# d8ahazard/AudioLab

Hardware: AMD Instinct MI355X
Metric: stems*realtime-factor (44.1kHz stereo) (higher is better)
Workload: dtype bf16; 1 GPU; MDX-Net UVR 4-stem (4x TFC-TDF U-Net L=11 g=48 dim_f=3072 dim_t=256 n_fft=6144), 300 s 44.1 kHz stereo in total, margin chunker, windows/launch=52; stems=4

## Files before the change

### audiolab_amd/csrc/tdfnet.hip

```cpp
#include "mma.h"
#include <alsep_gfx950_asm.h>

#include <map>
#include <type_traits>

namespace {

constexpr int kThreads = 256;

template <typename T> struct Vec16;
template <> struct Vec16<float> { static constexpr int N = 4; };
template <> struct Vec16<bf16_t> { static constexpr int N = 8; };
__device__ __forceinline__ void store_vec(float* p, const float* y) { *reinterpret_cast<float4*>(p) = make_float4(y[0], y[1], y[2], y[3]); }
__device__ __forceinline__ void store_vec(bf16_t* p, const float* y) {
    bf16x8 q;
#pragma unroll
    for (int e = 0; e < 8; ++e) q[e] = (bf16_t)y[e];
    *reinterpret_cast<bf16x8*>(p) = q;
}
__device__ __forceinline__ void load_vec(const float* p, float* x) {
    const float4 q = *reinterpret_cast<const float4*>(p);
    x[0] = q.x; x[1] = q.y; x[2] = q.z; x[3] = q.w;
}
__device__ __forceinline__ void load_vec(const bf16_t* p, float* x) {
// ... 2357 lines not shown
#pragma unroll
    for (int j = 0; j < P::D; ++j)
        if (j < nmy) issue(j);
    for (int i = 0; i < nmy; ++i) {
        pipe_wait_tile<P::D, P::ND, P::NS>(i, nmy);
        barrier_nodrain();
        if (i + P::D < nmy) issue(i + P::D);
        if (i > 0) copy_out(i - 1);
        const bf16_t* xs = reinterpret_cast<const bf16_t*>(xring + (size_t)(i % P::NSX) * P::x_bytes);
        f32x4 acc[P::MT][P::NI];
#pragma unroll
        for (int mt = 0; mt < P::MT; ++mt)
#pragma unroll
            for (int ni = 0; ni < P::NI; ++ni) acc[mt][ni] = f32x4{0.f, 0.f, 0.f, 0.f};
        bf16x8 xf[2][P::NI];
        static_for<P::NI>([&](auto nic) {
            constexpr int ni = decltype(nic)::value;
            lds_read_async_b128<ni * 2 * P::XREG>(xf[0][ni], xs + bk[0] / sizeof(bf16_t));
        });
        static_for<P::KS>([&](auto ksc) {
            constexpr int ks = decltype(ksc)::value, b = ks & 1;
            if constexpr (ks + 1 < P::KS) {
                static_for<P::NI>([&](auto nic) {
                    constexpr int ni = decltype(nic)::value;
                    lds_read_async_b128<ni * 2 * P::XREG>(xf[1 - b][ni], xs + bk[ks + 1] / sizeof(bf16_t));
                });
                lds_wait_n<P::NI>();
            } else {
                lds_wait_n<0>();
                if (P::C % 32 != 0) {
#pragma unroll
                    for (int ni = 0; ni < P::NI; ++ni) xf[b][ni] = klast_ok ? xf[b][ni] : bf16x8{};
                }
            }
#pragma unroll
            for (int mt = 0; mt < P::MT; ++mt)
#pragma unroll
                for (int ni = 0; ni < P::NI; ++ni) mma_step(acc[mt][ni], wf[mt][ks], xf[b][ni]);
        });
        bf16_t* sl = reinterpret_cast<bf16_t*>(sring + (size_t)(i % P::NSS) * P::s_bytes + ebase);
        const float* bnl = bn + 4 * lq;
        auto eoff = [&](int mt) {
            int t = 2 * mt + erot;
            t = t >= P::NG ? t - P::NG : t;
            return t * 8;
        };
        bf16x8 ev[2][P::NI];
        f32x4 scv[2], shv[2];
        auto eread = [&](auto mtc) {
            constexpr int mt = decltype(mtc)::value, eb = mt & 1;
            const bf16_t* p = sl + eoff(mt);
            static_for<P::NI>([&](auto nic) {
                constexpr int ni = decltype(nic)::value;
                lds_read_async_b128<ni * 32 * P::NG * 16>(ev[eb][ni], p);
            });
            lds_read_async_f32x4<0>(scv[eb], bnl + mt * 16);
            lds_read_async_f32x4<P::C2 * 4>(shv[eb], bnl + mt * 16);
        };
        eread(std::integral_constant<int, 0>{});
        static_for<P::MT>([&](auto mtc) {
            constexpr int mt = decltype(mtc)::value, b = mt & 1;
            if constexpr (mt + 1 < P::MT) {
                eread(std::integral_constant<int, mt + 1>{});
                lds_wait_n<P::NI + 2>();
            } else {
                lds_wait_n<0>();
            }
            bf16_t* p = sl + eoff(mt) + (lq & 1) * 4;
            static_for<P::NI>([&](auto nic) {
                constexpr int ni = decltype(nic)::value;
                const bf16x4 sk = (lq & 1) ? __builtin_shufflevector(ev[b][ni], ev[b][ni], 4, 5, 6, 7)
                                           : __builtin_shufflevector(ev[b][ni], ev[b][ni], 0, 1, 2, 3);
                bf16x4 q;
#pragma unroll
                for (int r = 0; r < 4; ++r) q[r] = (bf16_t)(fmaxf(fmaf(acc[mt][ni][r], scv[b][r], shv[b][r]), 0.f) * (float)sk[r]);
                lds_write_async_b64(p + ni * 32 * P::NG * 8, q);
            });
        });
    }
    barrier_nodrain();
    copy_out(nmy - 1);
}

template <int NM_, int TW_>
struct ConvAllco {
    static constexpr int NM = NM_, TW = TW_, TH = 8, KC = 48, CG = 6, NG = 54, NS = 14, NI = TW / 16, ROWS = 16 * NM, NB = NM, NPAIR = NB / 2;
    static constexpr int UPK = NM % 4 == 0 ? 4 : 3, G = NM / UPK;
    static constexpr int KS = 1, NSLOT = 4, DIST = NSLOT - 1, NSTG = NS / KS, UPS = UPK * KS;
    static constexpr int PW = TW + 2, PH = TH + 2;
    static constexpr int PGROUPS = PH * PW * CG, PINST = (PGROUPS + 63) / 64, PJ = (PINST + 7) / 8, PBUF = PINST * 64;
    static constexpr int KSTEP_BYTES = ROWS * 64, SLOT_BYTES = KS * KSTEP_BYTES;
    static constexpr int WPW = SLOT_BYTES / 8;
    static constexpr int WJ = (WPW + 1023) / 1024, WLAST = (WPW - (WJ - 1) * 1024) / 16;
    static constexpr int ST = NI * (NPAIR + NB % 2);
    static constexpr size_t ring_bytes = 16 * (size_t)(2 * PBUF) + (size_t)NSLOT * SLOT_BYTES;
    static constexpr size_t lds_bytes = ring_bytes + 2 * ROWS * sizeof(float) + 1024;
    static_assert(NM % 3 == 0 && NM % UPK == 0 && TW % 16 == 0 && NS % KS == 0 && SLOT_BYTES % (8 * 16) == 0, "ConvAllco: shape");
    static_assert(DIST >= 2 && DIST < NSTG && WJ < UPS && PJ - 1 <= NSTG - DIST && NSTG - 1 >= PJ, "ConvAllco: DMA schedule");
    static_assert(lds_bytes <= 160 * 1024, "ConvAllco: LDS budget");
    __host__ __device__ static constexpr int wswz(int row) { return ((row >> 3) & 1) << 1; }
    __host__ __device__ static constexpr int tapoff(int tap) { return ((tap / 3) * PW + tap % 3) * KC * 2; }
    __host__ __device__ static constexpr int xconst(int st) { return tapoff(4 * st / CG) + 16 * (4 * st % CG); }
    __host__ __device__ static constexpr int xkind(int st) { return st == 4 ? 1 : st == NS - 1 ? 2 : 0; }
    __host__ __device__ static constexpr int xbase(int kind, int wave, int l15, int lq) {
        const int a = (wave * PW + l15) * KC * 2 + 16 * lq;
        return kind == 0 ? a : kind == 1 ? a + (lq >= 2 ? (PW - 3) * KC * 2 : 0) : a - (lq >= 2 ? 16 * (lq - 1) : 0);
    }
    static_assert(CG == 6 && NS == 14 && NG == 54, "xconst / xkind are written for 54 groups in 14 k-steps");
    __host__ __device__ static constexpr int dma_of_stage(int sc) { return WJ + (sc < PJ ? 1 : 0); }
    __host__ __device__ static constexpr int inflight_at(int sc) {
        int n = 0;
        for (int i = 1; i <= DIST - 2; ++i) n += dma_of_stage((sc - i + NSTG) % NSTG);
        return n;
    }
};

template <typename Cf, int U>
__device__ __forceinline__ void allco_read_w(bf16x8 (&wf)[2][Cf::G], const bf16_t* wl) {
    constexpr int st = U / Cf::UPK, t = U % Cf::UPK;
    static_for<Cf::G>([&](auto gc) {
        constexpr int g = decltype(gc)::value;
        lds_read_async_b128<(t * Cf::G + g) * 1024 + (st % Cf::KS) * Cf::KSTEP_BYTES>(wf[U & 1][g], wl);
    });
}
template <typename Cf, int ST, int NI>
__device__ __forceinline__ void allco_read_x(bf16x8& xf, const bf16_t* pb) {
    lds_read_async_b128<NI * 16 * Cf::KC * 2 + Cf::xconst(ST)>(xf, pb);
}

template <int NM, int TW>
__global__ void __launch_bounds__(kBigThreads, 2)
conv3x3_bf16_allco_kernel(const bf16_t* __restrict__ X, bf16_t* __restrict__ Y, const bf16_t* __restrict__ Wp, const float* __restrict__ scale,
                          const float* __restrict__ shift, const bf16_t* __restrict__ zero_page, int Th, int Fw, int Cin, int Cout, int tiles_t,
                          int tiles_f, int ntiles) {
    typedef ConvAllco<NM, TW> Cf;
    bf16_t* const patch0 = reinterpret_cast<bf16_t*>(alsep_smem);
    bf16_t* const wring = patch0 + (size_t)2 * Cf::PBUF * 8;
    float* ss = reinterpret_cast<float*>(alsep_smem + Cf::ring_bytes);
    bf16_t* const scratch = reinterpret_cast<bf16_t*>(alsep_smem + Cf::lds_bytes - 1024);
    const int tid = threadIdx.x, lane = tid & 63, wave = __builtin_amdgcn_readfirstlane(tid >> 6);
    const int l15 = lane & 15, lq = lane >> 4;
    const int nq = Cin / Cf::KC;
    for (int i = tid; i < Cf::ROWS; i += kBigThreads) {
        ss[i] = scale[i];
        ss[Cf::ROWS + i] = shift[i];
    }
    __syncthreads();

    int xb[3];
#pragma unroll
    for (int kind = 0; kind < 3; ++kind) xb[kind] = Cf::xbase(kind, wave, l15, lq) / 2;
    const int wl_off = l15 * 32 + (lq ^ Cf::wswz(l15)) * 8;

    const int my_tiles = (ntiles - (int)blockIdx.x + (int)gridDim.x - 1) / (int)gridDim.x;
    const int npatch = my_tiles * nq;
    auto tile_coords = [&](int k, int& t0, int& f0, int64_t& b) {
        int tile = (int)blockIdx.x + k * (int)gridDim.x;
        const int tf = tile % tiles_f;  tile /= tiles_f;
        const int tt = tile % tiles_t;
        b = tile / tiles_t;
        t0 = tt * Cf::TH;
        f0 = tf * Cf::TW;
    };
    int prel[Cf::PJ];
    unsigned pflags[(Cf::PJ + 5) / 6] = {};
#pragma unroll
    for (int j = 0; j < Cf::PJ; ++j) {
        const int u = (wave + 8 * j) * 64 + lane;
        const int uu = u < Cf::PGROUPS ? u : Cf::PGROUPS - 1;
        const int P = uu / Cf::CG, cg = uu % Cf::CG;
        const int dt = P / Cf::PW - 1, df = P % Cf::PW - 1;
        prel[j] = (dt * Fw + df) * Cin + cg * 8;
        pflags[j / 6] |= (u < Cf::PGROUPS ? (unsigned)((dt < 0) | ((dt >= Cf::TH) << 1) | ((df < 0) << 2) | ((df >= Cf::TW) << 3)) : 16u) << (5 * (j % 6));
    }
    const bf16_t* psrc = X;
    unsigned pborder = 0;
    bf16_t* pdst = patch0;
    auto patch_prep = [&](int ps) {
        const int pc = ps < npatch ? ps : npatch - 1;
        int t0, f0; int64_t b;
        tile_coords(pc / nq, t0, f0, b);
        psrc = X + ((b * Th + t0) * (int64_t)Fw + f0) * Cin + (pc % nq) * Cf::KC;
        pborder = (unsigned)(t0 == 0) | ((unsigned)(t0 + Cf::TH >= Th) << 1) | ((unsigned)(f0 == 0) << 2) | ((unsigned)(f0 + Cf::TW >= Fw) << 3);
        pdst = patch0 + (size_t)(ps & 1) * Cf::PBUF * 8;
    };
    auto patch_one = [&](int j) {
        const int i = wave + 8 * j;
        const bool out = (pflags[j / 6] & ((pborder | 16u) << (5 * (j % 6)))) != 0;
        const bool real = j < Cf::PJ - 1 || i < Cf::PINST;
        const bf16_t* src = (out || !real) ? zero_page : psrc + opaque_vgpr(prel[j]);
        glds16(src, real ? pdst + (size_t)i * 64 * 8 : scratch);
    };
    const unsigned wlane = lane * 8;
    const bf16_t* wsrc_next = Wp;
    bf16_t* wdst_next = wring;
    auto weights_prep = [&](int q, int sc, int slot) {
        wsrc_next = Wp + ((size_t)q * Cf::NSTG + sc) * (Cf::SLOT_BYTES / 2) + wave * (Cf::WPW / 2);
        wdst_next = wring + (size_t)slot * (Cf::SLOT_BYTES / 2) + wave * (Cf::WPW / 2);
    };
    auto weights_one = [&](int j) {
        if (j < Cf::WJ - 1 || Cf::WLAST == 64 || lane < Cf::WLAST) glds16(wsrc_next + (wlane + j * 512u), wdst_next + j * 512);
    };

    f32x4 acc[Cf::NB][Cf::NI];
    bf16x8 xf[Cf::NI], wf[2][Cf::G];
    auto read_first = [&](const bf16_t* patch, const bf16_t* wl) {
        allco_read_w<Cf, 0>(wf, wl);
        static_for<Cf::NI>([&](auto nic) { allco_read_x<Cf, 0, decltype(nic)::value>(xf[decltype(nic)::value], patch + xb[0]); });
    };
    if (npatch > 0) {
        patch_prep(0);
#pragma unroll
        for (int j = 0; j < Cf::PJ; ++j) patch_one(j);
#pragma unroll
        for (int d = 0; d < Cf::DIST; ++d) {
            weights_prep(0, d, d);
#pragma unroll
            for (int j = 0; j < Cf::WJ; ++j) weights_one(j);
        }
        wait_vmcnt<0>();
        barrier_nodrain();
        read_first(patch0, wring + wl_off);
    }
    auto epilogue = [&](int k) {
        int t0, f0; int64_t b;
        tile_coords(k, t0, f0, b);
        const int le = opaque_vgpr(lane), l15 = le & 15, lq = le >> 4;
        bf16_t* yb = Y + ((b * Th + t0 + wave) * (int64_t)Fw + f0 + l15) * Cout;
#pragma unroll
        for (int j = 0; j < Cf::NPAIR; ++j) {
            const int co = j * 32 + lq * 8;
            f32x4 scv[2], shv[2];
#pragma unroll
            for (int h = 0; h < 2; ++h) {
                scv[h] = *reinterpret_cast<const f32x4*>(ss + co + 4 * h);
                shv[h] = *reinterpret_cast<const f32x4*>(ss + Cf::ROWS + co + 4 * h);
            }
#pragma unroll
            for (int ni = 0; ni < Cf::NI; ++ni) {
                float y[8];
#pragma unroll
                for (int h = 0; h < 2; ++h)
#pragma unroll
                    for (int r = 0; r < 4; ++r) y[4 * h + r] = fmaxf(fmaf(acc[2 * j + h][ni][r], scv[h][r], shv[h][r]), 0.f);
                store8(yb + (int64_t)ni * 16 * Cout + co, y);
            }
        }
        if constexpr (Cf::NB % 2 == 1) {
            constexpr int bb = Cf::NB - 1;
            const int co = bb * 16 + lq * 4;
            const f32x4 scv = *reinterpret_cast<const f32x4*>(ss + co);
            const f32x4 shv = *reinterpret_cast<const f32x4*>(ss + Cf::ROWS + co);
#pragma unroll
            for (int ni = 0; ni < Cf::NI; ++ni) {
                float y[4];
#pragma unroll
                for (int r = 0; r < 4; ++r) y[r] = fmaxf(fmaf(acc[bb][ni][r], scv[r], shv[r]), 0.f);
                store4(yb + (int64_t)ni * 16 * Cout + co, y);
            }
        }
    };

    int slot = 0, q = 0, k = 0;
    for (int p = 0; p < npatch; ++p) {
        const bf16_t* const patch = patch0 + (size_t)(p & 1) * Cf::PBUF * 8;
        const bf16_t* const patch_nx = patch0 + (size_t)((p + 1) & 1) * Cf::PBUF * 8;
        const int qn = q + 1 == nq ? 0 : q + 1;
        static_for<Cf::NSTG>([&](auto scc) {
            constexpr int sc = decltype(scc)::value;
            if (sc < Cf::DIST - 1 && q == 0 && p > 0) wait_vmcnt<Cf::inflight_at(sc) + Cf::ST>();
            else wait_vmcnt<Cf::inflight_at(sc)>();
            __builtin_amdgcn_s_barrier();
            const int slot_prev = slot == 0 ? Cf::NSLOT - 1 : slot - 1, slot_nx = slot + 1 == Cf::NSLOT ? 0 : slot + 1;
            weights_prep((sc + Cf::DIST) / Cf::NSTG ? qn : q, (sc + Cf::DIST) % Cf::NSTG, slot_prev);
            if (sc == 0) {
                patch_prep(p + 1);
                if (q == 0) {
#pragma unroll
                    for (int b = 0; b < Cf::NB; ++b)
#pragma unroll
                        for (int ni = 0; ni < Cf::NI; ++ni) acc[b][ni] = f32x4{0.f, 0.f, 0.f, 0.f};
                }
            }
            const bf16_t* const wl = wring + (size_t)slot * (Cf::SLOT_BYTES / 2) + wl_off;
            const bf16_t* const wl_nx = wring + (size_t)slot_nx * (Cf::SLOT_BYTES / 2) + wl_off;
            static_for<Cf::UPS>([&](auto uic) {
                constexpr int ui = decltype(uic)::value, U = sc * Cf::UPS + ui, t = U % Cf::UPK, st = U / Cf::UPK;
                constexpr bool chunk_end = U + 1 == Cf::UPK * Cf::NS;
                constexpr int U1 = chunk_end ? 0 : U + 1, st1 = U1 / Cf::UPK;
                if constexpr (t == 0) lds_wait_n<Cf::NI - 1>();
                else lds_wait_n<0>();
                if constexpr (!chunk_end) allco_read_w<Cf, U1>(wf, ui + 1 < Cf::UPS ? wl : wl_nx);
                if constexpr (t == 0) {
                    static_for<Cf::NI>([&](auto nic) {
                        constexpr int ni = decltype(nic)::value;
                        if constexpr (ni > 0) lds_wait_n<Cf::G + Cf::NI - 1 - ni>();
#pragma unroll
                        for (int g = 0; g < Cf::G; ++g) mma_step(acc[t * Cf::G + g][ni], wf[U & 1][g], xf[ni]);
                    });
                } else if constexpr (t == Cf::UPK - 1 && !chunk_end) {
                    const bf16_t* const pb = patch + xb[Cf::xkind(st1)];
                    static_for<Cf::NI>([&](auto nic) {
                        constexpr int ni = decltype(nic)::value;
#pragma unroll
                        for (int g = 0; g < Cf::G; ++g) mma_step(acc[t * Cf::G + g][ni], wf[U & 1][g], xf[ni]);
                        sched_fence();
                        allco_read_x<Cf, st1, ni>(xf[ni], pb);
                    });
                } else {
#pragma unroll
                    for (int g = 0; g < Cf::G; ++g)
#pragma unroll
                        for (int ni = 0; ni < Cf::NI; ++ni) mma_step(acc[t * Cf::G + g][ni], wf[U & 1][g], xf[ni]);
                }
                if constexpr (ui < Cf::WJ) weights_one(ui);
                if constexpr (ui == Cf::WJ && sc < Cf::PJ) patch_one(sc);
                sched_fence();
            });
            slot = slot_nx;
            if (sc == Cf::NSTG - 1 && q == nq - 1) epilogue(k);
        });
        read_first(patch_nx, wring + (size_t)slot * (Cf::SLOT_BYTES / 2) + wl_off);
        q = qn;
        if (q == 0) ++k;
    }
    lds_wait_n<0>();
    wait_vmcnt<0>();
}

#ifndef ALSEP_F16_TU
#include "tdfnet_f32s.h"
#endif

struct DevBuf {
    void* p = nullptr;
    size_t bytes = 0;
};

struct ConvLayer {
    DevBuf w, scale, shift;
    DevBuf w_big;
    DevBuf w_mq;
    DevBuf w_ac;
    int cin = 0, cout = 0;
    bool dma_path = false;
    int split = 0;
    unsigned* range_flag = nullptr;
};
struct GemmLayer {
    DevBuf w, bias, scale, shift;
    int M = 0, K = 0, Kp = 0, Mp = 0;
    bool has_bias = false;
    bool split = false;
    unsigned* range_flag = nullptr;
    bool dma_path = false;
    DevBuf wfrag;
    DevBuf wwide;
};
struct Block {
    std::vector<ConvLayer> tfc;
    std::vector<GemmLayer> tdf;
};

}

struct alsep_net {
    alsep_ctx* ctx = nullptr;
    alsep_net_config cfg{};
    int n = 0;
    bool split = false;
    DevBuf range_flag;
    std::vector<DevBuf> owned;
    DevBuf first_w, first_scale, first_shift, final_w, final_b, zero_page;
    std::vector<Block> enc, dec;
    Block bott;
    std::vector<GemmLayer> ds, us;
};

namespace {

typedef std::map<std::string, std::vector<float>> TensorMap;

template <typename T> T host_cast(float v);
template <> float host_cast<float>(float v) { return v; }
template <> bf16_t host_cast<bf16_t>(float v) { return (bf16_t)v; }

int upload(alsep_net* net, const void* src, size_t bytes, DevBuf* out) {
    void* d = nullptr;
    if (hipMalloc(&d, bytes ? bytes : 16) != hipSuccess) return alsep_fail(net->ctx, ALSEP_ERR_NOMEM, "hipMalloc(%zu) failed", bytes);
    out->p = d;
    out->bytes = bytes;
    net->owned.push_back(*out);
    if (bytes) ALSEP_HIP(net->ctx, hipMemcpy(d, src, bytes, hipMemcpyHostToDevice));
    return ALSEP_OK;
}

const std::vector<float>* find(const TensorMap& tm, const std::string& name, int64_t numel, alsep_ctx* ctx, bool required = true) {
    auto it = tm.find(name);
    if (it == tm.end()) {
        if (required) alsep_fail(ctx, ALSEP_ERR_ARG, "missing tensor '%s'", name.c_str());
        return nullptr;
    }
    if ((int64_t)it->second.size() != numel) {
        alsep_fail(ctx, ALSEP_ERR_ARG, "tensor '%s' has %zu elements, expected %lld", name.c_str(), it->second.size(), (long long)numel);
        return nullptr;
    }
    return &it->second;
// ... 54 lines not shown
    for (int R = 0; R < cout; ++R) std::copy(w.begin() + ConvBig<NY>::channel_of_row(R) * row, w.begin() + (ConvBig<NY>::channel_of_row(R) + 1) * row, wp.begin() + R * row);
    return pack_conv3x3_dma(wp, cin, cout);
}

std::vector<bf16_t> pack_conv3x3_mq(const std::vector<float>& w, int cin) {
    typedef ConvMq Cf;
    const int nq = cin / Cf::KC;
    std::vector<bf16_t> out((size_t)nq * Cf::PARTS * Cf::WGROUPS * 8, host_cast<bf16_t>(0.f));
    for (int q = 0; q < nq; ++q)
        for (int pt = 0; pt < Cf::PARTS; ++pt)
            for (int R = 0; R < Cf::ROWS; ++R)
                for (int stl = 0; stl < Cf::ksteps_of_part(pt); ++stl)
                    for (int lq = 0; lq < 4; ++lq) {
                        const int tap = pt * Cf::KS + stl, co = ConvBig<2>::channel_of_row(R);
                        const size_t dst = ((((size_t)q * Cf::PARTS + pt) * Cf::ROWS + R) * Cf::WG + 4 * stl + (lq ^ Cf::wswz(R))) * 8;
                        for (int e = 0; e < 8; ++e) {
                            const int ci = q * Cf::KC + lq * 8 + e;
                            out[dst + e] = host_cast<bf16_t>(w[(((size_t)co * cin + ci) * 3 + tap / 3) * 3 + tap % 3]);
                        }
                    }
    return out;
}

template <int NM>
std::vector<bf16_t> pack_conv3x3_allco(const std::vector<float>& w, int cin) {
    typedef ConvAllco<NM, 48> Cf;
    const int nq = cin / Cf::KC;
    std::vector<bf16_t> out((size_t)nq * Cf::NS * Cf::ROWS * 32, host_cast<bf16_t>(0.f));
    for (int q = 0; q < nq; ++q)
        for (int st = 0; st < Cf::NS; ++st)
            for (int R = 0; R < Cf::ROWS; ++R)
                for (int lq = 0; lq < 4; ++lq) {
                    const int grp = 4 * st + lq;
                    if (grp >= Cf::NG) continue;
                    const int tap = grp / Cf::CG, cg = grp % Cf::CG, co = ConvBig<NM / 3>::channel_of_row(R);
                    const size_t dst = ((((size_t)q * Cf::NS + st) * Cf::ROWS + R) * 4 + (lq ^ Cf::wswz(R))) * 8;
                    for (int e = 0; e < 8; ++e) {
                        const int ci = q * Cf::KC + cg * 8 + e;
                        out[dst + e] = host_cast<bf16_t>(w[(((size_t)co * cin + ci) * 3 + tap / 3) * 3 + tap % 3]);
                    }
                }
    return out;
}

template <typename T> constexpr bool is_bf16() { return false; }
template <> constexpr bool is_bf16<bf16_t>() { return true; }

template <typename T>
int make_conv(alsep_net* net, const TensorMap& tm, const std::string& p, int c, ConvLayer* L) {
    auto w = find(tm, p + ".weight", (int64_t)c * c * 9, net->ctx);
    auto sc = find(tm, p + ".scale", c, net->ctx);
    auto sh = find(tm, p + ".shift", c, net->ctx);
    if (!w || !sc || !sh) return ALSEP_ERR_ARG;
    L->cin = L->cout = c;
    int rc;
#ifndef ALSEP_F16_TU
    if (!is_bf16<T>() && net->split && (c % 48 == 0 || c % 16 == 0)) {
        L->split = c % 48 == 0 ? 24 : 16;
        L->range_flag = (unsigned*)net->range_flag.p;
        const std::vector<hs_t> pk = L->split == 24 ? pack_conv3x3_split<24, 48>(*w, c, c) : pack_conv3x3_split<16, 16>(*w, c, c);
        rc = upload(net, pk.data(), pk.size() * sizeof(hs_t), &L->w);
    } else
#endif
    if (is_bf16<T>() && c % 48 == 0) {
        L->dma_path = true;
        auto pk = pack_conv3x3_dma(*w, c, c);
        rc = upload(net, pk.data(), pk.size() * sizeof(bf16_t), &L->w);
        if (!rc && c == 48) {
            auto p0 = pack_conv3x3_big<1>(*w, c);
            rc = upload(net, p0.data(), p0.size() * sizeof(bf16_t), &L->w_big);
        }
        if (!rc && c == 96) {
            auto pq = pack_conv3x3_mq(*w, c);
            rc = upload(net, pq.data(), pq.size() * sizeof(bf16_t), &L->w_mq);
        }
        if (!rc && c == 144) {
            auto pb = pack_conv3x3_big<3>(*w, c);
            rc = upload(net, pb.data(), pb.size() * sizeof(bf16_t), &L->w_big);
        }
        if (!rc && c == 144) {
            auto pa = pack_conv3x3_allco<9>(*w, c);
            rc = upload(net, pa.data(), pa.size() * sizeof(bf16_t), &L->w_ac);
        }
    } else if (conv_uses_main<T>(c, c)) {
        auto pk = pack_conv3x3<T, ConvSel<T>::KC, ConvSel<T>::BN>(*w, c, c);
        rc = upload(net, pk.data(), pk.size() * sizeof(T), &L->w);
    } else {
        auto pk = pack_conv3x3<T, ConvSel16<T>::KC, ConvSel16<T>::BN>(*w, c, c);
        rc = upload(net, pk.data(), pk.size() * sizeof(T), &L->w);
    }
    if (rc) return rc;
    if ((rc = upload(net, sc->data(), c * sizeof(float), &L->scale))) return rc;
    return upload(net, sh->data(), c * sizeof(float), &L->shift);
}

template <typename T>
int make_gemm_weights(alsep_net* net, const std::vector<float>& wmk, int M, int K, GemmLayer* L) {
    typedef GemmCfg<T> Gc;
    L->M = M; L->K = K;
#ifndef ALSEP_F16_TU
    if (!is_bf16<T>() && net->split) {
        L->split = true;
        L->range_flag = (unsigned*)net->range_flag.p;
        const std::vector<hs_t> pk = pack_gemm_split(wmk, M, K, &L->Mp, &L->Kp);
        return upload(net, pk.data(), pk.size() * sizeof(hs_t), &L->w);
    }
#endif
    L->Mp = (int)ceil_div64(M, Gc::BR) * Gc::BR;
    L->Kp = (int)ceil_div64(K, Gc::BK) * Gc::BK;
    std::vector<T> pk((size_t)L->Mp * L->Kp, host_cast<T>(0.f));
    for (int m = 0; m < M; ++m)
        for (int k = 0; k < K; ++k) pk[(size_t)m * L->Kp + k] = host_cast<T>(wmk[(size_t)m * K + k]);
    return upload(net, pk.data(), pk.size() * sizeof(T), &L->w);
}

int make_tdf_dma_weights(alsep_net* net, const std::vector<float>& wmk, int M, int K, GemmLayer* L) {
    typedef TdfB16 Tc;
    L->M = M; L->K = K;
    L->Mp = (int)ceil_div64(M, Tc::BM) * Tc::BM;
    L->Kp = (int)ceil_div64(K, Tc::BK) * Tc::BK;
    L->dma_path = true;
    std::vector<bf16_t> pk((size_t)L->Mp * L->Kp, host_cast<bf16_t>(0.f));
    for (int m = 0; m < M; ++m)
        for (int kt = 0; kt < L->Kp / Tc::BK; ++kt)
            for (int g = 0; g < 8; ++g) {
                const int ks = g >> 2, lq = g & 3, pg = g ^ ((m >> 1) & 7);
                for (int e = 0; e < 8; ++e) {
                    const int k = kt * Tc::BK + ks * 32 + (e < 4 ? 4 * lq + e : 16 + 4 * lq + (e - 4));
                    if (k < K) pk[(size_t)m * L->Kp + kt * Tc::BK + pg * 8 + e] = host_cast<bf16_t>(wmk[(size_t)m * K + k]);
                }
            }
    return upload(net, pk.data(), pk.size() * sizeof(bf16_t), &L->w);
}

int make_tdf_wide_weights(alsep_net* net, const std::vector<float>& wmk, int M, int K, GemmLayer* L) {
    const int KT = (int)ceil_div64(K, 64);
    std::vector<bf16_t> pk((size_t)(M / 48) * KT * 6 * 512, host_cast<bf16_t>(0.f));
    for (int rb = 0; rb < M / 48; ++rb)
        for (int kt = 0; kt < KT; ++kt)
            for (int ks = 0; ks < 2; ++ks)
                for (int mi = 0; mi < 3; ++mi)
                    for (int l = 0; l < 64; ++l)
                        for (int e = 0; e < 8; ++e) {
                            const int lq = l >> 4, m = rb * 48 + mi * 16 + (l & 15);
                            const int k = kt * 64 + ks * 32 + (e < 4 ? 4 * lq + e : 16 + 4 * lq + (e - 4));
                            if (k < K)
                                pk[((((size_t)rb * KT + kt) * 2 + ks) * 3 + mi) * 512 + l * 8 + e] =
                                    host_cast<bf16_t>(wmk[(size_t)m * K + k]);
                        }
    return upload(net, pk.data(), pk.size() * sizeof(bf16_t), &L->wwide);
}

int make_frag_weights(alsep_net* net, const std::vector<float>& wmk, int M, int K, DevBuf* out) {
    const int MT = (M + 15) / 16, KS = (K + 31) / 32;
    std::vector<bf16_t> pk((size_t)MT * KS * 64 * 8, host_cast<bf16_t>(0.f));
    for (int mt = 0; mt < MT; ++mt)
        for (int ks = 0; ks < KS; ++ks)
            for (int l = 0; l < 64; ++l)
                for (int e = 0; e < 8; ++e) {
                    const int m = mt * 16 + (l & 15), k = ks * 32 + (l >> 4) * 8 + e;
                    if (m < M && k < K) pk[(((size_t)mt * KS + ks) * 64 + l) * 8 + e] = host_cast<bf16_t>(wmk[(size_t)m * K + k]);
                }
    return upload(net, pk.data(), pk.size() * sizeof(bf16_t), out);
}

template <typename T>
// ... 131 lines not shown
    typedef ConvB16<TW> Cf;
    const int tiles_t = (int)ceil_div64(Th, Cf::TH), tiles_f = (int)ceil_div64(Fw, TW);
    const int64_t ntiles = B * tiles_t * tiles_f;
    if (ntiles > 0x7fffffff) return alsep_fail(ctx, ALSEP_ERR_ARG, "conv3x3: too many tiles");
    ALSEP_HIP(ctx, hipFuncSetAttribute((const void*)conv3x3_bf16_kernel<TW>, hipFuncAttributeMaxDynamicSharedMemorySize,
                                       (int)Cf::lds_bytes));
    ProfScope prof(ctx, TW == 64 ? ALSEP_PROF_CONV3X3 : ALSEP_PROF_CONV3X3_SMALL);
    prof.work(18.0 * (double)L.cin * L.cout * B * Th * Fw, (double)sizeof(*X) * B * Th * Fw * (L.cin + L.cout));
    const int nyc = L.cout / Cf::BN;
    const int ny_fastest = conv_ny_fastest() && ntiles % 8 == 0 && nyc > 1 && ntiles * nyc <= 0x7fffffff;
    hipLaunchKernelGGL((conv3x3_bf16_kernel<TW>), ny_fastest ? dim3((unsigned)(ntiles * nyc)) : dim3((unsigned)ntiles, nyc),
                       dim3(kThreads), Cf::lds_bytes,
                       ctx->stream, X, Y, (const bf16_t*)L.w.p, (const float*)L.scale.p, (const float*)L.shift.p, zero_page,
                       Th, Fw, L.cin, L.cout, tiles_t, tiles_f, (int)ntiles,  0,  0, ny_fastest);
    note_launch(ctx, TW == 64 ? "conv3x3_bf16_kernel<64>" : "conv3x3_bf16_kernel<small>");
    ALSEP_LAUNCH_CHECK(ctx, "conv3x3_bf16_kernel");
    return ALSEP_OK;
}

template <int NQ, int RING_ = 3, int OCC = 1, int TW_ = 64>
int launch_conv_regw(alsep_ctx* ctx, const ConvLayer& L, const bf16_t* X, bf16_t* Y, const bf16_t* zero_page, int64_t B,
                     int Th, int Fw) {
    typedef ConvRW<NQ, RING_, TW_> Cf;
    const int tiles_t = Th / Cf::TH, tiles_f = Fw / Cf::TW;
    const int64_t ntiles = B * tiles_t * tiles_f;
    if (ntiles > 0x7fffffff) return alsep_fail(ctx, ALSEP_ERR_ARG, "conv3x3: too many tiles");
    ALSEP_HIP(ctx, hipFuncSetAttribute((const void*)conv3x3_bf16_regw_kernel<NQ, RING_, OCC, TW_>,
                                       hipFuncAttributeMaxDynamicSharedMemorySize, (int)Cf::lds_bytes));
    const int ny = L.cout / Cf::BN;
    int gx = OCC * 256 / ny;
    if (gx > ntiles) gx = (int)ntiles;
    ProfScope prof(ctx, ALSEP_PROF_CONV3X3_REGW);
    prof.work(18.0 * (double)L.cin * L.cout * B * Th * Fw, (double)sizeof(*X) * B * Th * Fw * (L.cin + L.cout));
    hipLaunchKernelGGL((conv3x3_bf16_regw_kernel<NQ, RING_, OCC, TW_>), dim3((unsigned)gx, ny), dim3(kThreads), Cf::lds_bytes, ctx->stream, X, Y,
                       (const bf16_t*)L.w.p, (const float*)L.scale.p, (const float*)L.shift.p, zero_page, Th, Fw, L.cin,
                       L.cout, tiles_t, tiles_f, (int)ntiles);
    ALSEP_LAUNCH_CHECK(ctx, "conv3x3_bf16_regw_kernel");
    return ALSEP_OK;
}

template <typename Cf, typename Kern>
int launch_conv_persist(alsep_ctx* ctx, Kern kern, const ConvLayer& L, const DevBuf& wimg, int prof_class, const char* name, const bf16_t* X,
                        bf16_t* Y, const bf16_t* zero_page, int64_t B, int Th, int Fw, int grid_cap = 0) {
    const int tiles_t = Th / Cf::TH, tiles_f = Fw / Cf::TW;
    const int64_t ntiles = B * tiles_t * tiles_f;
    if (ntiles > 0x7fffffff) return alsep_fail(ctx, ALSEP_ERR_ARG, "conv3x3: too many tiles");
    ALSEP_HIP(ctx, hipFuncSetAttribute((const void*)kern, hipFuncAttributeMaxDynamicSharedMemorySize, (int)Cf::lds_bytes));
    int gx = ntiles < 256 ? (int)ntiles : 256;
    if (grid_cap > 0 && gx > grid_cap) gx = grid_cap;
    ProfScope prof(ctx, prof_class);
    prof.work(18.0 * (double)L.cin * L.cout * B * Th * Fw, (double)sizeof(*X) * B * Th * Fw * (L.cin + L.cout));
    hipLaunchKernelGGL(kern, dim3((unsigned)gx), dim3(kBigThreads), Cf::lds_bytes, ctx->stream, X, Y, (const bf16_t*)wimg.p,
                       (const float*)L.scale.p, (const float*)L.shift.p, zero_page, Th, Fw, L.cin, L.cout, tiles_t, tiles_f, (int)ntiles);
    ALSEP_LAUNCH_CHECK(ctx, name);
    return ALSEP_OK;
}

int launch_conv_big3(alsep_ctx* ctx, const ConvLayer& L, const bf16_t* X, bf16_t* Y, const bf16_t* zero_page, int64_t B, int Th, int Fw) {
    if (!L.w_big.p) return alsep_fail(ctx, ALSEP_ERR_STATE, "conv3x3: no big-tile weight image for this layer");
    if (int rc = launch_conv_persist<ConvBig<3>>(ctx, conv3x3_bf16_big_kernel<3>, L, L.w_big, ALSEP_PROF_CONV3X3_BIG3, "conv3x3_bf16_big_kernel",
                                                 X, Y, zero_page, B, Th, Fw))
        return rc;
    note_launch(ctx, "conv3x3_bf16_big_kernel<3>");
    return ALSEP_OK;
}

int launch_conv_mq(alsep_ctx* ctx, const ConvLayer& L, const bf16_t* X, bf16_t* Y, const bf16_t* zero_page, int64_t B, int Th, int Fw) {
    if (!L.w_mq.p || L.cout != ConvMq::ROWS || L.cin % ConvMq::KC) return alsep_fail(ctx, ALSEP_ERR_STATE, "conv3x3: no mq weight image for this layer");
    return launch_conv_persist<ConvMq>(ctx, conv3x3_bf16_mq_kernel, L, L.w_mq, ALSEP_PROF_CONV3X3_BIG, "conv3x3_bf16_mq_kernel", X, Y, zero_page,
                                       B, Th, Fw);
}

int launch_conv_m0(alsep_ctx* ctx, const ConvLayer& L, const bf16_t* X, bf16_t* Y, const bf16_t* zero_page, int64_t B, int Th, int Fw) {
    if (!L.w_big.p || L.cout != ConvM0::ROWS || L.cin != ConvM0::KC) return alsep_fail(ctx, ALSEP_ERR_STATE, "conv3x3: no m0 weight image for this layer");
    return launch_conv_persist<ConvM0>(ctx, conv3x3_bf16_m0_kernel, L, L.w_big, ALSEP_PROF_CONV3X3_REGW, "conv3x3_bf16_m0_kernel", X, Y, zero_page,
                                       B, Th, Fw);
}

int conv_allco_grid() {
    static const int v = env_int("ALSEP_CONV_ALLCO_GRID", 0);
    return v;
}

template <int NM>
int launch_conv_allco(alsep_ctx* ctx, const ConvLayer& L, const bf16_t* X, bf16_t* Y, const bf16_t* zero_page, int64_t B, int Th, int Fw) {
    typedef ConvAllco<NM, 48> Cf;
    if (!L.w_ac.p || L.cout != Cf::ROWS || L.cin != L.cout) return alsep_fail(ctx, ALSEP_ERR_STATE, "conv3x3: no all-channels weight image for this layer");
    static_assert(NM == 9, "only the c = 144 instance is shipped: the profiling class and the names below are level 2's");
    if (int rc = launch_conv_persist<Cf>(ctx, conv3x3_bf16_allco_kernel<NM, 48>, L, L.w_ac, ALSEP_PROF_CONV3X3_BIG3, "conv3x3_bf16_allco_kernel", X, Y,
                                         zero_page, B, Th, Fw, conv_allco_grid()))
        return rc;
    note_launch(ctx, "conv3x3_bf16_big_kernel");
    note_launch(ctx, "conv3x3_bf16_big_kernel<3>");
    return ALSEP_OK;
}

int conv_m0_enabled() {
    static const int v = env_int("ALSEP_CONV_M0", 1);
    return v;
}
int conv_regw_enabled() {
    static const int v = env_int("ALSEP_CONV_REGW", 1);
    return v;
}
int conv_big_enabled() {
    static const int v = env_int("ALSEP_CONV_BIG", 1);
    return v;
}
int conv_mq_enabled() {
    static const int v = env_int("ALSEP_CONV_MQ", 1);
    return v;
}
int conv_big3_enabled() {
    static const int v = env_int("ALSEP_CONV_BIG3", 1);
    return v;
}

int conv_allco_enabled() {
    static const int v = env_int("ALSEP_CONV_ALLCO", 1);
    return v;
}
constexpr int kConvAllco144 = 1;
constexpr int kConvAllcoRouted = kConvAllco144;

int run_conv_dma(alsep_ctx* ctx, const ConvLayer& L, const bf16_t* X, bf16_t* Y, const bf16_t* zp, int64_t B, int Th, int Fw) {
    if (conv_m0_enabled() && L.cin == 48 && L.cout == 48 && Th % 8 == 0 && Fw % 48 == 0 &&
        (conv_m0_enabled() >= 2 || B * (Th / 8) * (Fw / 48) >= 256))
        return launch_conv_m0(ctx, L, X, Y, zp, B, Th, Fw);
    if (conv_regw_enabled() && Th % 4 == 0 && Fw % 64 == 0 && L.cin == L.cout) {
        if (L.cin == 48 && conv_regw_enabled() == 3) return launch_conv_regw<1>(ctx, L, X, Y, zp, B, Th, Fw);
        if (L.cin == 48) return launch_conv_regw<1, 3, 2, 32>(ctx, L, X, Y, zp, B, Th, Fw);
        if (L.cin == 96 && conv_regw_enabled() >= 2) return launch_conv_regw<2>(ctx, L, X, Y, zp, B, Th, Fw);
    }
    if (conv_big_enabled() && conv_big3_enabled() && conv_allco_enabled() && Th % 8 == 0 && Fw % 48 == 0 && L.cin == 144 && L.cout == 144) {
        const int mode = conv_allco_enabled();
        const bool big3_shape = Fw % 64 == 0 && (conv_big_enabled() >= 2 || B * (Th / 8) * (Fw / 64) >= 96);
        if (mode >= 2 || ((kConvAllcoRouted & kConvAllco144) && big3_shape)) return launch_conv_allco<9>(ctx, L, X, Y, zp, B, Th, Fw);
    }
    if (conv_big_enabled() && Th % 8 == 0 && Fw % 64 == 0 && L.cin == L.cout &&
        (conv_big_enabled() >= 2 || B * (Th / 8) * (Fw / 64) >= 96)) {
        if (L.cout == 96 && conv_mq_enabled()) return launch_conv_mq(ctx, L, X, Y, zp, B, Th, Fw);
        if (L.cout == 144 && conv_big3_enabled()) return launch_conv_big3(ctx, L, X, Y, zp, B, Th, Fw);
    }
    if (Fw >= 64 && Fw % 64 == 0) return launch_conv_dma<64>(ctx, L, X, Y, zp, B, Th, Fw);
    if (Fw >= 32) return launch_conv_dma<32>(ctx, L, X, Y, zp, B, Th, Fw);
    return launch_conv_dma<16>(ctx, L, X, Y, zp, B, Th, Fw);
}
int run_conv_dma(alsep_ctx* ctx, const ConvLayer&, const float*, float*, const float*, int64_t, int, int) {
    return alsep_fail(ctx, ALSEP_ERR_STATE, "LDS-DMA conv path is bf16 only");
}

#ifndef ALSEP_F16_TU
template <int KC, int BN, int TW>
int launch_conv_split(alsep_ctx* ctx, const ConvLayer& L, const float* X, float* Y, int64_t B, int Th, int Fw) {
    typedef ConvSCfg<KC, BN, TW> Cf;
    const int tiles_t = (int)ceil_div64(Th, Cf::TH), tiles_f = (int)ceil_div64(Fw, TW);
    const int64_t ntiles = B * tiles_t * tiles_f;
    const int nyc = L.cout / BN;
    if (ntiles * nyc > 0x7fffffff) return alsep_fail(ctx, ALSEP_ERR_ARG, "conv3x3: too many tiles");
    ALSEP_HIP(ctx, hipFuncSetAttribute((const void*)conv3x3_f32s_kernel<KC, BN, TW>, hipFuncAttributeMaxDynamicSharedMemorySize,
                                       (int)Cf::lds_bytes));
    ProfScope prof(ctx, TW >= 32 ? ALSEP_PROF_CONV3X3 : ALSEP_PROF_CONV3X3_SMALL);
    prof.work(18.0 * (double)L.cin * L.cout * B * Th * Fw, 4.0 * B * Th * Fw * (L.cin + L.cout));
    const int nyf = (ntiles % 8 == 0 && nyc > 1) ? 1 : 0;
    const dim3 grid = nyf ? dim3((unsigned)(ntiles * nyc)) : dim3((unsigned)ntiles, nyc);
    hipLaunchKernelGGL((conv3x3_f32s_kernel<KC, BN, TW>), grid, dim3(kThreads), Cf::lds_bytes, ctx->stream, X, Y,
                       (const hs_t*)L.w.p, (const float*)L.scale.p, (const float*)L.shift.p, Th, Fw, L.cin, L.cout, tiles_t, tiles_f,
                       (int)ntiles, nyf, L.range_flag);
    ALSEP_LAUNCH_CHECK(ctx, "conv3x3_f32s_kernel");
    return ALSEP_OK;
}
template <int KC, int BN>
int run_conv_split_tw(alsep_ctx* ctx, const ConvLayer& L, const float* X, float* Y, int64_t B, int Th, int Fw) {
    if (Fw >= 32) return launch_conv_split<KC, BN, 32>(ctx, L, X, Y, B, Th, Fw);
    return launch_conv_split<KC, BN, 16>(ctx, L, X, Y, B, Th, Fw);
}
int run_conv_split(alsep_ctx* ctx, const ConvLayer& L, const float* X, float* Y, int64_t B, int Th, int Fw) {
    return L.split == 24 ? run_conv_split_tw<24, 48>(ctx, L, X, Y, B, Th, Fw) : run_conv_split_tw<16, 16>(ctx, L, X, Y, B, Th, Fw);
}
int run_conv_split(alsep_ctx* ctx, const ConvLayer&, const bf16_t*, bf16_t*, int64_t, int, int) {
    return alsep_fail(ctx, ALSEP_ERR_STATE, "split contraction is a float32 mode");
}
#endif

template <typename T>
int run_conv(alsep_ctx* ctx, const ConvLayer& L, const T* X, T* Y, int64_t B, int Th, int Fw, const void* zero_page) {
#ifndef ALSEP_F16_TU
    if (L.split) return run_conv_split(ctx, L, X, Y, B, Th, Fw);
#endif
    if (L.dma_path) return run_conv_dma(ctx, L, X, Y, (const T*)zero_page, B, Th, Fw);
    if (conv_uses_main<T>(L.cin, L.cout)) return run_conv_tw<T, ConvSel<T>::KC, ConvSel<T>::BN>(ctx, L, X, Y, B, Th, Fw);
    return run_conv_tw<T, ConvSel16<T>::KC, ConvSel16<T>::BN>(ctx, L, X, Y, B, Th, Fw);
}

int pix_stream_enabled() {
    static const int v = env_int("ALSEP_PIX_STREAM", 1);
    return v;
}
enum { kPixPipeDs96 = 1, kPixPipeDs144 = 2, kPixPipeUs192 = 4, kPixPipeUs144 = 8 };
constexpr int kPixPipeRouted = kPixPipeDs96 | kPixPipeDs144 | kPixPipeUs192 | kPixPipeUs144;
bool pix_pipe_routed(int kind) {
    static const int v = env_int("ALSEP_PIX_PIPE", 1);
    return v >= 2 || (v == 1 && (kPixPipeRouted & kind));
}
unsigned pix_pipe_grid(alsep_ctx* ctx, int64_t ntile) {
    static const int cap = env_int("ALSEP_PIX_PIPE_GRID", 0);
    int64_t grid = device_cu_count(ctx);
    if (cap > 0 && cap < grid) grid = cap;
    return (unsigned)std::min<int64_t>(grid, ntile);
}
template <int C_, int PX_, int D_>
hipError_t launch_ds_pipe(alsep_ctx* ctx, const GemmLayer& L, const bf16_t* X, bf16_t* Y, int64_t ncols, int Tp, int Fp) {
    typedef DsPipeCfg<C_, PX_, D_> P;
    const hipError_t e = hipFuncSetAttribute((const void*)ds_pipe_kernel<C_, PX_, D_>, hipFuncAttributeMaxDynamicSharedMemorySize, (int)P::lds_bytes);
    if (e != hipSuccess) return e;
    hipLaunchKernelGGL((ds_pipe_kernel<C_, PX_, D_>), dim3(pix_pipe_grid(ctx, ncols / P::PX)), dim3(kThreads), P::lds_bytes, ctx->stream, X, Y,
                       (const bf16_t*)L.wfrag.p, (const float*)L.scale.p, (const float*)L.shift.p, ncols, Tp, Fp);
    return hipSuccess;
}
template <int CIN, int C2_, int NI_, int D_>
// ... 533 lines not shown
```

Baseline: 6337 stems*x_realtime.

## Extend all-channels persistent conv3x3 kernel to 192/288 channels via output groups

Generalizes the all-output-channels persistent conv3x3 kernel with an NGRP parameter, so a tile iterates over several 96-channel output groups while reusing the same patch staging and weight DMA pipeline. Weights for c=192 and c=288 are packed per group. The c=192 layer is routed to the new kernel by default with a 64-wide tile. The intent is to replace the generic conv path at those levels with the pipelined LDS-DMA kernel. The cost is that each input patch is re-staged once per output group, and the change adds template instances and extra weight images.

```diff
diff --git a/audiolab_amd/csrc/tdfnet.hip b/audiolab_amd/csrc/tdfnet.hip
--- a/audiolab_amd/csrc/tdfnet.hip
+++ b/audiolab_amd/csrc/tdfnet.hip
@@ -2463,8 +2463,9 @@
     copy_out(nmy - 1);
 }
 
-template <int NM_, int TW_>
+template <int NM_, int TW_, int NGRP_ = 1>
 struct ConvAllco {
+    static constexpr int NGRP = NGRP_, COUT = NGRP_ * 16 * NM_;
     static constexpr int NM = NM_, TW = TW_, TH = 8, KC = 48, CG = 6, NG = 54, NS = 14, NI = TW / 16, ROWS = 16 * NM, NB = NM, NPAIR = NB / 2;
     static constexpr int UPK = NM % 4 == 0 ? 4 : 3, G = NM / UPK;
     static constexpr int KS = 1, NSLOT = 4, DIST = NSLOT - 1, NSTG = NS / KS, UPS = UPK * KS;
@@ -2475,8 +2476,8 @@
     static constexpr int WJ = (WPW + 1023) / 1024, WLAST = (WPW - (WJ - 1) * 1024) / 16;
     static constexpr int ST = NI * (NPAIR + NB % 2);
     static constexpr size_t ring_bytes = 16 * (size_t)(2 * PBUF) + (size_t)NSLOT * SLOT_BYTES;
-    static constexpr size_t lds_bytes = ring_bytes + 2 * ROWS * sizeof(float) + 1024;
-    static_assert(NM % 3 == 0 && NM % UPK == 0 && TW % 16 == 0 && NS % KS == 0 && SLOT_BYTES % (8 * 16) == 0, "ConvAllco: shape");
+    static constexpr size_t lds_bytes = ring_bytes + 2 * COUT * sizeof(float) + 1024;
+    static_assert(NGRP >= 1 && NM % 3 == 0 && NM % UPK == 0 && TW % 16 == 0 && NS % KS == 0 && SLOT_BYTES % (8 * 16) == 0, "ConvAllco: shape");
     static_assert(DIST >= 2 && DIST < NSTG && WJ < UPS && PJ - 1 <= NSTG - DIST && NSTG - 1 >= PJ, "ConvAllco: DMA schedule");
     static_assert(lds_bytes <= 160 * 1024, "ConvAllco: LDS budget");
     __host__ __device__ static constexpr int wswz(int row) { return ((row >> 3) & 1) << 1; }
@@ -2509,12 +2510,12 @@
     lds_read_async_b128<NI * 16 * Cf::KC * 2 + Cf::xconst(ST)>(xf, pb);
 }
 
-template <int NM, int TW>
+template <int NM, int TW, int NGRP>
 __global__ void __launch_bounds__(kBigThreads, 2)
 conv3x3_bf16_allco_kernel(const bf16_t* __restrict__ X, bf16_t* __restrict__ Y, const bf16_t* __restrict__ Wp, const float* __restrict__ scale,
                           const float* __restrict__ shift, const bf16_t* __restrict__ zero_page, int Th, int Fw, int Cin, int Cout, int tiles_t,
                           int tiles_f, int ntiles) {
-    typedef ConvAllco<NM, TW> Cf;
+    typedef ConvAllco<NM, TW, NGRP> Cf;
     bf16_t* const patch0 = reinterpret_cast<bf16_t*>(alsep_smem);
     bf16_t* const wring = patch0 + (size_t)2 * Cf::PBUF * 8;
     float* ss = reinterpret_cast<float*>(alsep_smem + Cf::ring_bytes);
@@ -2522,9 +2523,9 @@
     const int tid = threadIdx.x, lane = tid & 63, wave = __builtin_amdgcn_readfirstlane(tid >> 6);
     const int l15 = lane & 15, lq = lane >> 4;
     const int nq = Cin / Cf::KC;
-    for (int i = tid; i < Cf::ROWS; i += kBigThreads) {
+    for (int i = tid; i < Cf::COUT; i += kBigThreads) {
         ss[i] = scale[i];
-        ss[Cf::ROWS + i] = shift[i];
+        ss[Cf::COUT + i] = shift[i];
     }
     __syncthreads();
 
@@ -2534,7 +2535,7 @@
     const int wl_off = l15 * 32 + (lq ^ Cf::wswz(l15)) * 8;
 
     const int my_tiles = (ntiles - (int)blockIdx.x + (int)gridDim.x - 1) / (int)gridDim.x;
-    const int npatch = my_tiles * nq;
+    const int npatch = my_tiles * Cf::NGRP * nq;
     auto tile_coords = [&](int k, int& t0, int& f0, int64_t& b) {
         int tile = (int)blockIdx.x + k * (int)gridDim.x;
         const int tf = tile % tiles_f;  tile /= tiles_f;
@@ -2560,7 +2561,7 @@
     auto patch_prep = [&](int ps) {
         const int pc = ps < npatch ? ps : npatch - 1;
         int t0, f0; int64_t b;
-        tile_coords(pc / nq, t0, f0, b);
+        tile_coords(pc / nq / Cf::NGRP, t0, f0, b);
         psrc = X + ((b * Th + t0) * (int64_t)Fw + f0) * Cin + (pc % nq) * Cf::KC;
         pborder = (unsigned)(t0 == 0) | ((unsigned)(t0 + Cf::TH >= Th) << 1) | ((unsigned)(f0 == 0) << 2) | ((unsigned)(f0 + Cf::TW >= Fw) << 3);
         pdst = patch0 + (size_t)(ps & 1) * Cf::PBUF * 8;
@@ -2575,8 +2576,9 @@
     const unsigned wlane = lane * 8;
     const bf16_t* wsrc_next = Wp;
     bf16_t* wdst_next = wring;
-    auto weights_prep = [&](int q, int sc, int slot) {
-        wsrc_next = Wp + ((size_t)q * Cf::NSTG + sc) * (Cf::SLOT_BYTES / 2) + wave * (Cf::WPW / 2);
+    auto weights_prep = [&](int g, int q, int sc, int slot) {
+        const int gq = Cf::NGRP > 1 ? g * nq + q : q;
+        wsrc_next = Wp + ((size_t)gq * Cf::NSTG + sc) * (Cf::SLOT_BYTES / 2) + wave * (Cf::WPW / 2);
         wdst_next = wring + (size_t)slot * (Cf::SLOT_BYTES / 2) + wave * (Cf::WPW / 2);
     };
     auto weights_one = [&](int j) {
@@ -2595,7 +2597,7 @@
         for (int j = 0; j < Cf::PJ; ++j) patch_one(j);
 #pragma unroll
         for (int d = 0; d < Cf::DIST; ++d) {
-            weights_prep(0, d, d);
+            weights_prep(0, 0, d, d);
 #pragma unroll
             for (int j = 0; j < Cf::WJ; ++j) weights_one(j);
         }
@@ -2603,19 +2605,21 @@
         barrier_nodrain();
         read_first(patch0, wring + wl_off);
     }
-    auto epilogue = [&](int k) {
+    auto epilogue = [&](int k, int g) {
         int t0, f0; int64_t b;
         tile_coords(k, t0, f0, b);
         const int le = opaque_vgpr(lane), l15 = le & 15, lq = le >> 4;
-        bf16_t* yb = Y + ((b * Th + t0 + wave) * (int64_t)Fw + f0 + l15) * Cout;
+        const int c0 = Cf::NGRP > 1 ? g * Cf::ROWS : 0;
+        bf16_t* yb = Y + ((b * Th + t0 + wave) * (int64_t)Fw + f0 + l15) * Cout + c0;
+        const float* const ssg = ss + c0;
 #pragma unroll
         for (int j = 0; j < Cf::NPAIR; ++j) {
             const int co = j * 32 + lq * 8;
             f32x4 scv[2], shv[2];
 #pragma unroll
             for (int h = 0; h < 2; ++h) {
-                scv[h] = *reinterpret_cast<const f32x4*>(ss + co + 4 * h);
-                shv[h] = *reinterpret_cast<const f32x4*>(ss + Cf::ROWS + co + 4 * h);
+                scv[h] = *reinterpret_cast<const f32x4*>(ssg + co + 4 * h);
+                shv[h] = *reinterpret_cast<const f32x4*>(ssg + Cf::COUT + co + 4 * h);
             }
 #pragma unroll
             for (int ni = 0; ni < Cf::NI; ++ni) {
@@ -2630,8 +2634,8 @@
         if constexpr (Cf::NB % 2 == 1) {
             constexpr int bb = Cf::NB - 1;
             const int co = bb * 16 + lq * 4;
-            const f32x4 scv = *reinterpret_cast<const f32x4*>(ss + co);
-            const f32x4 shv = *reinterpret_cast<const f32x4*>(ss + Cf::ROWS + co);
+            const f32x4 scv = *reinterpret_cast<const f32x4*>(ssg + co);
+            const f32x4 shv = *reinterpret_cast<const f32x4*>(ssg + Cf::COUT + co);
 #pragma unroll
             for (int ni = 0; ni < Cf::NI; ++ni) {
                 float y[4];
@@ -2642,18 +2646,19 @@
         }
     };
 
-    int slot = 0, q = 0, k = 0;
+    int slot = 0, q = 0, k = 0, g = 0;
     for (int p = 0; p < npatch; ++p) {
         const bf16_t* const patch = patch0 + (size_t)(p & 1) * Cf::PBUF * 8;
         const bf16_t* const patch_nx = patch0 + (size_t)((p + 1) & 1) * Cf::PBUF * 8;
         const int qn = q + 1 == nq ? 0 : q + 1;
+        const int gn = Cf::NGRP > 1 && qn == 0 ? (g + 1 == Cf::NGRP ? 0 : g + 1) : g;
         static_for<Cf::NSTG>([&](auto scc) {
             constexpr int sc = decltype(scc)::value;
             if (sc < Cf::DIST - 1 && q == 0 && p > 0) wait_vmcnt<Cf::inflight_at(sc) + Cf::ST>();
             else wait_vmcnt<Cf::inflight_at(sc)>();
             __builtin_amdgcn_s_barrier();
             const int slot_prev = slot == 0 ? Cf::NSLOT - 1 : slot - 1, slot_nx = slot + 1 == Cf::NSLOT ? 0 : slot + 1;
-            weights_prep((sc + Cf::DIST) / Cf::NSTG ? qn : q, (sc + Cf::DIST) % Cf::NSTG, slot_prev);
+            weights_prep((sc + Cf::DIST) / Cf::NSTG ? gn : g, (sc + Cf::DIST) / Cf::NSTG ? qn : q, (sc + Cf::DIST) % Cf::NSTG, slot_prev);
             if (sc == 0) {
                 patch_prep(p + 1);
                 if (q == 0) {
@@ -2699,11 +2704,12 @@
                 sched_fence();
             });
             slot = slot_nx;
-            if (sc == Cf::NSTG - 1 && q == nq - 1) epilogue(k);
+            if (sc == Cf::NSTG - 1 && q == nq - 1) epilogue(k, g);
         });
         read_first(patch_nx, wring + (size_t)slot * (Cf::SLOT_BYTES / 2) + wl_off);
         q = qn;
-        if (q == 0) ++k;
+        g = gn;
+        if (q == 0 && g == 0) ++k;
     }
     lds_wait_n<0>();
     wait_vmcnt<0>();
@@ -2924,6 +2930,15 @@
             auto pa = pack_conv3x3_allco<9>(*w, c);
             rc = upload(net, pa.data(), pa.size() * sizeof(bf16_t), &L->w_ac);
         }
+        if (!rc && (c == 192 || c == 288)) {
+            std::vector<bf16_t> pa;
+            const size_t slice = (size_t)96 * c * 9;
+            for (int g = 0; g < c / 96; ++g) {
+                auto pg = pack_conv3x3_allco<6>(std::vector<float>(w->begin() + g * slice, w->begin() + (g + 1) * slice), c);
+                pa.insert(pa.end(), pg.begin(), pg.end());
+            }
+            rc = upload(net, pa.data(), pa.size() * sizeof(bf16_t), &L->w_ac);
+        }
     } else if (conv_uses_main<T>(c, c)) {
         auto pk = pack_conv3x3<T, ConvSel<T>::KC, ConvSel<T>::BN>(*w, c, c);
         rc = upload(net, pk.data(), pk.size() * sizeof(T), &L->w);
@@ -3221,16 +3236,25 @@
     return v;
 }
 
-template <int NM>
+template <int NM, int TW, int NGRP>
 int launch_conv_allco(alsep_ctx* ctx, const ConvLayer& L, const bf16_t* X, bf16_t* Y, const bf16_t* zero_page, int64_t B, int Th, int Fw) {
-    typedef ConvAllco<NM, 48> Cf;
-    if (!L.w_ac.p || L.cout != Cf::ROWS || L.cin != L.cout) return alsep_fail(ctx, ALSEP_ERR_STATE, "conv3x3: no all-channels weight image for this layer");
-    static_assert(NM == 9, "only the c = 144 instance is shipped: the profiling class and the names below are level 2's");
-    if (int rc = launch_conv_persist<Cf>(ctx, conv3x3_bf16_allco_kernel<NM, 48>, L, L.w_ac, ALSEP_PROF_CONV3X3_BIG3, "conv3x3_bf16_allco_kernel", X, Y,
+    typedef ConvAllco<NM, TW, NGRP> Cf;
+    static_assert((NM == 9 && TW == 48 && NGRP == 1) || (NM == 6 && NGRP >= 2), "an instance that has a weight image, names and a class below");
+    if (!L.w_ac.p || L.cout != Cf::COUT || L.cin != L.cout || Th % Cf::TH || Fw % TW)
+        return alsep_fail(ctx, ALSEP_ERR_STATE, "conv3x3: no all-channels weight image for this layer, or not its shape");
+    const bool plain64 = Fw >= 64 && Fw % 64 == 0;
+    const int prof_class = NGRP == 1 ? ALSEP_PROF_CONV3X3_BIG3 : plain64 ? ALSEP_PROF_CONV3X3 : ALSEP_PROF_CONV3X3_SMALL;
+    if (int rc = launch_conv_persist<Cf>(ctx, conv3x3_bf16_allco_kernel<NM, TW, NGRP>, L, L.w_ac, prof_class, "conv3x3_bf16_allco_kernel", X, Y,
                                          zero_page, B, Th, Fw, conv_allco_grid()))
         return rc;
-    note_launch(ctx, "conv3x3_bf16_big_kernel");
-    note_launch(ctx, "conv3x3_bf16_big_kernel<3>");
+    if (NGRP == 1) {
+        note_launch(ctx, "conv3x3_bf16_big_kernel");
+        note_launch(ctx, "conv3x3_bf16_big_kernel<3>");
+    } else {
+        note_launch(ctx, TW == 48 ? "conv3x3_bf16_allco_kernel<6,48>" : "conv3x3_bf16_allco_kernel<6,64>");
+        note_launch(ctx, "conv3x3_bf16_kernel");
+        note_launch(ctx, plain64 ? "conv3x3_bf16_kernel<64>" : "conv3x3_bf16_kernel<small>");
+    }
     return ALSEP_OK;
 }
 
@@ -3259,8 +3283,13 @@
     static const int v = env_int("ALSEP_CONV_ALLCO", 1);
     return v;
 }
-constexpr int kConvAllco144 = 1;
-constexpr int kConvAllcoRouted = kConvAllco144;
+constexpr int kConvAllco144 = 1, kConvAllco192 = 2;
+constexpr int kConvAllcoRouted = kConvAllco144 | kConvAllco192;
+constexpr int kConvAllcoTw = 64;
+int conv_allco_tw() {
+    static const int v = env_int("ALSEP_CONV_ALLCO_TW", kConvAllcoTw) == 48 ? 48 : 64;
+    return v;
+}
 
 int run_conv_dma(alsep_ctx* ctx, const ConvLayer& L, const bf16_t* X, bf16_t* Y, const bf16_t* zp, int64_t B, int Th, int Fw) {
     if (conv_m0_enabled() && L.cin == 48 && L.cout == 48 && Th % 8 == 0 && Fw % 48 == 0 &&
@@ -3274,7 +3303,15 @@
     if (conv_big_enabled() && conv_big3_enabled() && conv_allco_enabled() && Th % 8 == 0 && Fw % 48 == 0 && L.cin == 144 && L.cout == 144) {
         const int mode = conv_allco_enabled();
         const bool big3_shape = Fw % 64 == 0 && (conv_big_enabled() >= 2 || B * (Th / 8) * (Fw / 64) >= 96);
-        if (mode >= 2 || ((kConvAllcoRouted & kConvAllco144) && big3_shape)) return launch_conv_allco<9>(ctx, L, X, Y, zp, B, Th, Fw);
+        if (mode >= 2 || ((kConvAllcoRouted & kConvAllco144) && big3_shape)) return launch_conv_allco<9, 48, 1>(ctx, L, X, Y, zp, B, Th, Fw);
+    }
+    if (conv_big_enabled() && conv_allco_enabled() && L.cin == L.cout && (L.cout == 192 || L.cout == 288)) {
+        const int mode = conv_allco_enabled(), tw = conv_allco_tw();
+        const bool measured_shape = L.cout == 192 && Fw % 64 == 0 && (conv_big_enabled() >= 2 || B * (Th / 8) * (Fw / 64) >= 96);
+        if (Th % 8 == 0 && Fw % tw == 0 && (mode >= 2 || ((kConvAllcoRouted & kConvAllco192) && measured_shape))) {
+            if (L.cout == 192) return tw == 48 ? launch_conv_allco<6, 48, 2>(ctx, L, X, Y, zp, B, Th, Fw) : launch_conv_allco<6, 64, 2>(ctx, L, X, Y, zp, B, Th, Fw);
+            return tw == 48 ? launch_conv_allco<6, 48, 3>(ctx, L, X, Y, zp, B, Th, Fw) : launch_conv_allco<6, 64, 3>(ctx, L, X, Y, zp, B, Th, Fw);
+        }
     }
     if (conv_big_enabled() && Th % 8 == 0 && Fw % 64 == 0 && L.cin == L.cout &&
         (conv_big_enabled() >= 2 || B * (Th / 8) * (Fw / 64) >= 96)) {
```

Result: faster. 6510 stems*x_realtime, median of 6 (+2.7%).
